# Yifei-Y/Openset-RCNN

Measured on AMD Instinct MI355X. Metric: images/sec at 3x800x1333, R50-FPN, 1/2/4/8 MI355X; mAP_k vs ref, higher is better.
Workload: dtype f16; 1 GPU; VOC-COCO openset_rcnn_R50_FPN_128k.yaml, inference-only, 3x800x1333 uint8 BGR -> padded 800x1344, 1000 proposals/level (4273/img), 1000 dets/img, 50+50 final; batch_per_gpu=16, global_batch=16, parallelism=dp1 (images sharded, no collective), detections_last_step=1600, unknown_detections_last_step=800, known_detections_last_step=800, micro_batch_streams=1, hipgraph=True, ranks=1, distinct_gpus=1, passes_in_flight=4, images_in_flight=64

## Files before the change

### include/osr.h

```cpp
#ifndef OSR_H_
#define OSR_H_

#include <stdint.h>

#ifdef __cplusplus
extern "C" {
#endif

#define OSR_ABI_VERSION 1

typedef int32_t osr_status;
enum {
    OSR_OK = 0,
    OSR_ERR_INVALID_ARG = -1,
    OSR_ERR_UNSUPPORTED = -2,
    OSR_ERR_LAUNCH = -3,
    OSR_ERR_WORKSPACE = -4
};

typedef enum { OSR_F32 = 0, OSR_F16 = 1, OSR_BF16 = 2 } osr_dtype;

#define OSR_MAX_LEVELS 8

int32_t osr_abi_version(void);
// ... 137 lines not shown

int32_t osr_rpn_select_capacity(const osr_rpn_levels* lv, int32_t pre_nms_topk);
int64_t osr_rpn_select_workspace_bytes(const osr_rpn_levels* lv, int32_t n, int32_t pre_nms_topk);
osr_status osr_rpn_select(const osr_rpn_levels* lv, const float* cell_anchors , const float* ctr,
                          const float* deltas, int32_t n, const int32_t* image_hw , int32_t pre_nms_topk,
                          float min_box_size, float* boxes, float* scores, int32_t* src_index, int32_t* batch_idx,
                          int32_t* counts, int32_t* status_flags, void* workspace, int64_t workspace_bytes,
                          void* stream);

osr_status osr_rpn_select_ex(const osr_rpn_levels* lv, const float* cell_anchors, const float* ctr, const float* deltas,
                             int32_t n, const int32_t* image_hw, int32_t pre_nms_topk, float min_box_size,
                             int32_t decode_mode, const float reg_weights[4], float* boxes, float* scores,
                             int32_t* src_index, int32_t* batch_idx, int32_t* level_out, int32_t* counts,
                             int32_t* status_flags, void* workspace, int64_t workspace_bytes, void* stream);

typedef struct osr_pyramid {
    int32_t num_levels;
    int32_t c;
    int32_t h[OSR_MAX_LEVELS];
    int32_t w[OSR_MAX_LEVELS];
    float scale[OSR_MAX_LEVELS];
    const void* data[OSR_MAX_LEVELS];
} osr_pyramid;

osr_status osr_roi_align_fwd(const osr_pyramid* feats, int32_t feat_dtype, int32_t n, const float* boxes,
                             const int32_t* batch_idx, int64_t m, int32_t pooled, int32_t canonical_level,
                             int32_t canonical_size, int32_t min_level, void* out, int32_t out_dtype, void* stream);

osr_status osr_roi_align_fwd_ordered(const osr_pyramid* feats, int32_t feat_dtype, int32_t n, const float* boxes,
                                     const int32_t* batch_idx, int64_t m, int32_t pooled, int32_t canonical_level,
                                     int32_t canonical_size, int32_t min_level, const int32_t* order,
                                     const int32_t* order_nvalid, void* out, int32_t out_dtype, void* stream);
#define OSR_ROI_NO_PADDING_FILL 1
osr_status osr_roi_align_fwd_ordered_ex(const osr_pyramid* feats, int32_t feat_dtype, int32_t n, const float* boxes,
                                        const int32_t* batch_idx, int64_t m, int32_t pooled, int32_t canonical_level,
                                        int32_t canonical_size, int32_t min_level, const int32_t* order,
                                        const int32_t* order_nvalid, int32_t flags, void* out, int32_t out_dtype, void* stream);
#define OSR_ROI_MAX_SAMPLING_RATIO 64
typedef struct osr_roi_options {
    int32_t aligned;
    int32_t sampling_ratio;
} osr_roi_options;
osr_status osr_roi_align_fwd_ordered_opt(const osr_pyramid* feats, int32_t feat_dtype, int32_t n, const float* boxes,
                                         const int32_t* batch_idx, int64_t m, int32_t pooled, int32_t canonical_level,
                                         int32_t canonical_size, int32_t min_level, const int32_t* order,
                                         const int32_t* order_nvalid, int32_t flags, const osr_roi_options* options, void* out,
                                         int32_t out_dtype, void* stream);
int64_t osr_roi_locality_order_workspace_bytes(int32_t n, int64_t m);
osr_status osr_roi_locality_order(const osr_pyramid* feats, int32_t n, const float* boxes, const int32_t* batch_idx, int64_t m,
                                  int32_t canonical_level, int32_t canonical_size, int32_t min_level, int32_t* order,
                                  int32_t* nvalid, void* workspace, int64_t workspace_bytes, void* stream);

osr_status osr_box_predictor_tail(const float* x, int64_t m, int32_t k, const float* w, const float* b,
                                  const float* proposals, const float* ctr, const int32_t* batch_idx,
                                  const int32_t* image_hw, const float reg_weights[4], int32_t mean_type,
                                  float score_thresh, float* pred_deltas, float* pred_iou, float* boxes,
                                  float* score, int32_t* cand, void* stream);

int64_t osr_nms_topk_workspace_bytes(int32_t num_segments, int64_t seg_stride);
osr_status osr_nms_topk(const float* boxes, const float* scores, const int32_t* cls ,
                        const int32_t* cand , int32_t num_segments, int64_t seg_stride,
                        const int32_t* seg_len, float thr, int32_t topk, int32_t* keep, int32_t* keep_count,
                        void* workspace, int64_t workspace_bytes, void* stream);

osr_status osr_gather_rows(const float* src, int64_t seg_stride, int32_t row_elems, const int32_t* keep,
                           const int32_t* keep_count, int32_t num_segments, int32_t topk, float* dst, void* stream);
// ... 272 lines not shown
```

### openset-rcnn_amd/csrc/osr_roi_align.hip

```cpp
#include "osr_common.h"
#include <stdlib.h>

#ifndef RA_MAXC
#define RA_MAXC 32
#endif
#ifndef RA_MAXX
#define RA_MAXX 192
#endif
#ifndef RA_FWD_MAXX
#define RA_FWD_MAXX 96
#endif
#ifndef RA_PAIR
#define RA_PAIR 0
#endif
#ifndef RA_PD1
#define RA_PD1 6
#define RA_PD2 4
#define RA_PD3 2
#define RA_PD4 2
#endif
#ifndef RA_SD1
#define RA_SD1 8
#define RA_SD2 4
#define RA_SD3 3
// ... 2 lines not shown
#endif
#define RA_MAXD 16

struct RaOpt {
    float off;
    int clamp1;
    int sgrid;
};

static bool ra_opt_default(const osr_roi_options* o) { return !o || (o->aligned == 1 && o->sampling_ratio == 0); }
static RaOpt ra_opt_of(const osr_roi_options* o) {
    RaOpt r;
    r.off = (!o || o->aligned) ? 0.5f : 0.f; r.clamp1 = (o && !o->aligned) ? 1 : 0; r.sgrid = o ? o->sampling_ratio : 0;
    return r;
}
#define RA_REQUIRE_OPT(o, name)                                                                                                              \
    OSR_REQUIRE(!(o) || (o)->aligned == 0 || (o)->aligned == 1, OSR_ERR_INVALID_ARG, name ": options: aligned must be 0 or 1, got %d", (o)->aligned); \
    OSR_REQUIRE(!(o) || ((o)->sampling_ratio >= 0 && (o)->sampling_ratio <= OSR_ROI_MAX_SAMPLING_RATIO), OSR_ERR_INVALID_ARG,               \
                name ": options: sampling_ratio must be 0 (adaptive) .. %d, got %d", OSR_ROI_MAX_SAMPLING_RATIO, (o)->sampling_ratio)

struct RoiAlignArgs {
    const void* data[4];
    int h[4], w[4];
    float scale[4];
    int num_levels, c;
    const float* boxes;
    const int* batch_idx;
    long long m;
    int pooled, canonical_level, canonical_size, min_level;
    void* out;
    const int* order;
    const int* order_nvalid;
    int no_pad_fill;
    RaOpt opt;
};

template <class T> struct Vec4;
template <> struct Vec4<float> { typedef float4 type; };
template <> struct Vec4<f16_t> { typedef uint2 type; };
template <> struct Vec4<bf16_t> { typedef uint2 type; };

template <class T> __device__ __forceinline__ void load4(const T* p, float v[4]);
template <> __device__ __forceinline__ void load4<float>(const float* p, float v[4]) {
    float4 t = *reinterpret_cast<const float4*>(p);
    v[0] = t.x; v[1] = t.y; v[2] = t.z; v[3] = t.w;
}
template <> __device__ __forceinline__ void load4<f16_t>(const f16_t* p, float v[4]) {
    typedef f16_t h4 __attribute__((ext_vector_type(4)));
    h4 t = *reinterpret_cast<const h4*>(p);
    v[0] = (float)t[0]; v[1] = (float)t[1]; v[2] = (float)t[2]; v[3] = (float)t[3];
}
template <> __device__ __forceinline__ void load4<bf16_t>(const bf16_t* p, float v[4]) {
    uint2 t = *reinterpret_cast<const uint2*>(p);
    v[0] = __uint_as_float(t.x << 16); v[1] = __uint_as_float(t.x & 0xffff0000u);
    v[2] = __uint_as_float(t.y << 16); v[3] = __uint_as_float(t.y & 0xffff0000u);
}
template <class T> __device__ __forceinline__ void store4(T* p, const float v[4]);
template <> __device__ __forceinline__ void store4<float>(float* p, const float v[4]) {
    *reinterpret_cast<float4*>(p) = make_float4(v[0], v[1], v[2], v[3]);
}
template <> __device__ __forceinline__ void store4<f16_t>(f16_t* p, const float v[4]) {
    typedef f16_t h4 __attribute__((ext_vector_type(4)));
    h4 t = {(f16_t)v[0], (f16_t)v[1], (f16_t)v[2], (f16_t)v[3]};
    *reinterpret_cast<h4*>(p) = t;
}
template <> __device__ __forceinline__ void store4<bf16_t>(bf16_t* p, const float v[4]) {
// ... 169 lines not shown
template <int D, class G, class LoadF, class ConsF>
__device__ __forceinline__ void ra_stream(int n, LoadF load, ConsF cons) {
    G v[D], u[D > 1 ? D - 1 : 1];
    const int q = n / D, r = n - q * D;
    if (q >= 1) {
#pragma unroll
        for (int d = 0; d < D; ++d) load(v[d], d);
        for (int i = 0; i + 1 < q; ++i) {
#pragma unroll
            for (int d = 0; d < D; ++d) { cons(v[d], i * D + d); load(v[d], (i + 1) * D + d); }
        }
    }
#pragma unroll
    for (int d = 0; d < D - 1; ++d) if (d < r) load(u[d], q * D + d);
    if (q >= 1) {
#pragma unroll
        for (int d = 0; d < D; ++d) cons(v[d], (q - 1) * D + d);
    }
#pragma unroll
    for (int d = 0; d < D - 1; ++d) if (d < r) cons(u[d], q * D + d);
}

template <class TO>
__device__ __forceinline__ void ra_store_bins(const ra_f2 (&acc)[7][2], float inv_count, TO* __restrict__ outrow, size_t ostride, bool cok, int P) {
    if (!cok) return;
#pragma unroll
    for (int b = 0; b < 7; ++b)
        if (b < P) {
            const float tot[4] = {acc[b][0][0] * inv_count, acc[b][0][1] * inv_count, acc[b][1][0] * inv_count, acc[b][1][1] * inv_count};
            store4<TO>(outrow + (size_t)b * ostride, tot);
        }
}

template <int NY, class TI, class TO>
__device__ __forceinline__ void ra_bin_row(__amdgpu_buffer_rsrc_t rs, int voff, int base, int istride_b, int sstride_b, int ncol, const RaWaveLds& S,
                                           const float (&wy)[6], float inv_count, TO* __restrict__ outrow, size_t ostride, bool cok, int P) {
    constexpr int D = NY == 1 ? RA_SD1 : NY == 2 ? RA_SD2 : NY == 3 ? RA_SD3 : NY <= 5 ? RA_SD4 : RA_SD6;
    static_assert(D <= RA_MAXD, "S.wfull is padded with RA_MAXD zero rows");
    ra_f2 acc[7][2];
#pragma unroll
    for (int b = 0; b < 7; ++b) { acc[b][0] = ra_f2{0.f, 0.f}; acc[b][1] = ra_f2{0.f, 0.f}; }
    struct Grp { Buf4<TI> p[NY]; };
    ra_stream<D, Grp>(
        ncol,
        [&](Grp& g, int x) {
            const int so = base + x * sstride_b;
#pragma unroll
            for (int j = 0; j < NY; ++j) g.p[j].load(rs, voff, so + j * istride_b);
        },
        [&](Grp& g, int x) {
            ra_f2 c0 = ra_f2{0.f, 0.f}, c1 = ra_f2{0.f, 0.f};
#pragma unroll
            for (int j = 0; j < NY; ++j) {
                ra_f2 lo, hi;
                g.p[j].get(lo, hi);
                const ra_f2 wj = ra_f2{wy[j], wy[j]};
                c0 = __builtin_elementwise_fma(wj, lo, c0);
                c1 = __builtin_elementwise_fma(wj, hi, c1);
            }
            const float4 wa = *reinterpret_cast<const float4*>(&S.wfull[x][0]), wb = *reinterpret_cast<const float4*>(&S.wfull[x][4]);
            const float wv[7] = {wa.x, wa.y, wa.z, wa.w, wb.x, wb.y, wb.z};
#pragma unroll
            for (int b = 0; b < 7; ++b) {
                const ra_f2 wq = ra_f2{wv[b], wv[b]};
                acc[b][0] = __builtin_elementwise_fma(wq, c0, acc[b][0]);
                acc[b][1] = __builtin_elementwise_fma(wq, c1, acc[b][1]);
            }
        });
    ra_store_bins<TO>(acc, inv_count, outrow, ostride, cok, P);
}

template <class T> struct Buf8;
template <int HI, bool FIRST> __device__ __forceinline__ float ra_mix(unsigned packed, float w, float c) {
    float d;
    if (FIRST) {
        if (HI) asm("v_fma_mix_f32 %0, %1, %2, 0 op_sel:[1,0,0] op_sel_hi:[1,0,0]" : "=v"(d) : "v"(packed), "s"(w));
        else asm("v_fma_mix_f32 %0, %1, %2, 0 op_sel_hi:[1,0,0]" : "=v"(d) : "v"(packed), "s"(w));
    } else {
        if (HI) asm("v_fma_mix_f32 %0, %1, %2, %3 op_sel:[1,0,0] op_sel_hi:[1,0,0]" : "=v"(d) : "v"(packed), "s"(w), "v"(c));
        else asm("v_fma_mix_f32 %0, %1, %2, %3 op_sel_hi:[1,0,0]" : "=v"(d) : "v"(packed), "s"(w), "v"(c));
    }
    return d;
}
template <> struct Buf8<f16_t> {
    ra_u32x4 r;
    __device__ __forceinline__ void load(__amdgpu_buffer_rsrc_t rs, int vo, int so) { r = __builtin_amdgcn_raw_buffer_load_b128(rs, vo, so, 0); }
    template <bool FIRST> __device__ __forceinline__ void fma_into(float w, float (&cs)[8]) const {
        _Pragma("unroll") for (int i = 0; i < 4; ++i) {
            cs[2 * i] = ra_mix<0, FIRST>(r[i], w, cs[2 * i]);
            cs[2 * i + 1] = ra_mix<1, FIRST>(r[i], w, cs[2 * i + 1]);
        }
    }
};
template <> struct Buf8<bf16_t> {
    ra_u32x4 r;
    __device__ __forceinline__ void load(__amdgpu_buffer_rsrc_t rs, int vo, int so) { r = __builtin_amdgcn_raw_buffer_load_b128(rs, vo, so, 0); }
    template <bool FIRST> __device__ __forceinline__ void fma_into(float w, float (&cs)[8]) const {
        _Pragma("unroll") for (int i = 0; i < 4; ++i) {
            cs[2 * i] = __builtin_fmaf(__uint_as_float(r[i] << 16), w, FIRST ? 0.f : cs[2 * i]);
            cs[2 * i + 1] = __builtin_fmaf(__uint_as_float(r[i] & 0xffff0000u), w, FIRST ? 0.f : cs[2 * i + 1]);
        }
// ... 24 lines not shown
            for (int j = 0; j < NY; ++j) g.p[j].load(rs, voff, so + j * istride_b);
        },
        [&](Grp& g, int ws) {
            float cs[8];
            g.p[0].template fma_into<true>(wy[0], cs);
#pragma unroll
            for (int j = 1; j < NY; ++j) g.p[j].template fma_into<false>(wy[j], cs);
            const float* wr = &S.wfull[2 * ws + half][0];
            const float4 wa = *reinterpret_cast<const float4*>(wr), wb = *reinterpret_cast<const float4*>(wr + 4);
            const float wv[7] = {wa.x, wa.y, wa.z, wa.w, wb.x, wb.y, wb.z};
#pragma unroll
            for (int b = 0; b < 7; ++b) {
                const ra_f2 wq = ra_f2{wv[b], wv[b]};
#pragma unroll
                for (int q = 0; q < 4; ++q) acc[b][q] = __builtin_elementwise_fma(wq, ra_f2{cs[2 * q], cs[2 * q + 1]}, acc[b][q]);
            }
        });
#pragma unroll
    for (int k2 = 0; k2 < 4; ++k2) {
        float tot[8];
#pragma unroll
        for (int q = 0; q < 4; ++q)
#pragma unroll
            for (int e = 0; e < 2; ++e) {
                const unsigned x = __float_as_uint(acc[2 * k2][q][e]), y = 2 * k2 + 1 < 7 ? __float_as_uint(acc[(2 * k2 + 1) % 7][q][e]) : 0u;
                const auto sw = __builtin_amdgcn_permlane32_swap(x, y, false, false);
                tot[2 * q + e] = (__uint_as_float(sw[0]) + __uint_as_float(sw[1])) * inv_count;
            }
        const int bin = 2 * k2 + half;
        if (cok && bin < P) store8<TO>(outrow + (size_t)bin * ostride, tot);
    }
}

template <class TI, class TO>
__device__ __forceinline__ void ra_bin_row_tall(__amdgpu_buffer_rsrc_t rs, int voff, int base, int istride_b, int sstride_b, int ncol, const RaWaveLds& S,
                                                const float* wrow, int ny, float inv_count, TO* __restrict__ outrow, size_t ostride, bool cok, int P) {
    ra_f2 acc[7][2];
#pragma unroll
    for (int b = 0; b < 7; ++b) { acc[b][0] = ra_f2{0.f, 0.f}; acc[b][1] = ra_f2{0.f, 0.f}; }
    for (int x = 0; x < ncol; ++x) {
        const int so = base + x * sstride_b;
        ra_f2 c0 = ra_f2{0.f, 0.f}, c1 = ra_f2{0.f, 0.f};
        for (int j0 = 0; j0 < ny; j0 += 6) {
            Buf4<TI> v[6];
#pragma unroll
            for (int j = 0; j < 6; ++j) v[j].load(rs, voff, so + min(j0 + j, ny - 1) * istride_b);
#pragma unroll
            for (int j = 0; j < 6; ++j) {
                ra_f2 lo, hi;
                v[j].get(lo, hi);
                const float w1 = j0 + j < ny ? wrow[j0 + j] : 0.f;
                const ra_f2 wj = ra_f2{w1, w1};
                c0 = __builtin_elementwise_fma(wj, lo, c0);
                c1 = __builtin_elementwise_fma(wj, hi, c1);
            }
        }
#pragma unroll
        for (int b = 0; b < 7; ++b) {
            const float w1 = S.wfull[x][b];
            const ra_f2 wq = ra_f2{w1, w1};
            acc[b][0] = __builtin_elementwise_fma(wq, c0, acc[b][0]);
            acc[b][1] = __builtin_elementwise_fma(wq, c1, acc[b][1]);
        }
    }
    ra_store_bins<TO>(acc, inv_count, outrow, ostride, cok, P);
}

#ifndef RA_GATHER_MAXS
#define RA_GATHER_MAXS 3
#endif
#ifndef RA_GATHER_BIN
#define RA_GATHER_BIN 2.0f
#endif
static_assert(RA_GATHER_MAXS >= 2 && RA_GATHER_MAXS <= 3, "gather instantiations exist for S = 1, 2 and 3");
static_assert(4 * RA_GATHER_MAXS <= RA_MAXC, "the taps of a bin are laid over its RA_MAXC table columns");
template <int SG, class TI, class TO>
__device__ __forceinline__ void ra_gather_roi(__amdgpu_buffer_rsrc_t rs, int lane, int sub, int C, int P, int W, const RaWaveLds& S,
                                              float inv_count, TO* __restrict__ out) {
    constexpr int NYG = SG <= 2 ? SG : 1;
    const int pix_b = C * (int)sizeof(TI), row_b = W * pix_b;
    for (int ph = sub; ph < P; ph += RA_WPR) {
        int yo[SG][2]; float wy[SG][2];
#pragma unroll
        for (int i = 0; i < SG; ++i)
#pragma unroll
            for (int t = 0; t < 2; ++t) {
                yo[i][t] = __builtin_amdgcn_readfirstlane(__float_as_int(S.w[0][ph][4 * i + t])) * row_b;
                wy[i][t] = __uint_as_float(__builtin_amdgcn_readfirstlane(__float_as_uint(S.w[0][ph][4 * i + 2 + t])));
            }
        for (int pw = 0; pw < P; ++pw) {
            int xo[SG][2]; float wx[SG][2];
#pragma unroll
            for (int i = 0; i < SG; ++i)
#pragma unroll
                for (int t = 0; t < 2; ++t) {
                    xo[i][t] = __builtin_amdgcn_readfirstlane(__float_as_int(S.w[1][pw][4 * i + t])) * pix_b;
                    wx[i][t] = __uint_as_float(__builtin_amdgcn_readfirstlane(__float_as_uint(S.w[1][pw][4 * i + 2 + t])));
// ... 160 lines not shown
    if (lane < P) {
#pragma unroll
        for (int ax = 0; ax < 2; ++ax) {
            const int lo = S.lo[ax][lane], n = S.n[ax][lane];
            if (n > 0) { lo_l[ax] = lo; hi_l[ax] = lo + n; }
        }
    }
#pragma unroll
    for (int ax = 0; ax < 2; ++ax)
#pragma unroll
        for (int d = 1; d < 8; d <<= 1) {
            lo_l[ax] = min(lo_l[ax], __shfl_xor(lo_l[ax], d, 64));
            hi_l[ax] = max(hi_l[ax], __shfl_xor(hi_l[ax], d, 64));
        }
    int ext_lo[2], ext_n[2];
    bool ax_ok[2];
#pragma unroll
    for (int ax = 0; ax < 2; ++ax) {
        const int l = __builtin_amdgcn_readfirstlane(lo_l[ax]), h = __builtin_amdgcn_readfirstlane(hi_l[ax]);
        ext_lo[ax] = l == 0x7fffffff ? 0 : l;
        ext_n[ax] = l == 0x7fffffff ? 0 : h - l;
        ax_ok[ax] = !fallback && ext_n[ax] <= RA_FWD_MAXX;
    }
    const unsigned long long lvl_bytes = (unsigned long long)H * W * C * sizeof(TI);
#ifndef RA_AXIS_SELECT
#define RA_AXIS_SELECT 1
#endif
    int oa = (!RA_AXIS_SELECT || ext_n[1] <= ext_n[0]) ? 1 : 0;
    if (!ax_ok[oa]) oa ^= 1;

    if (ax_ok[oa] && lvl_bytes < (1ull << 31)) {
        const int ia = oa ^ 1;
        const int os = ext_lo[oa], nstep = ext_n[oa];
        for (int sl = gtid; sl < nstep + RA_MAXD; sl += RA_WPR * 64) {
            const int x = os + sl;
#pragma unroll
            for (int bb = 0; bb < 8; ++bb) {
                float wv = 0.f;
                if (bb < P && sl < nstep) { const int i = x - S.lo[oa][bb]; if (i >= 0 && i < S.n[oa][bb]) wv = S.w[oa][bb][i]; }
                S.wfull[sl][bb] = wv;
            }
        }
        RA_SYNC();
        const float inv_count = 1.0f / count;
        const __amdgpu_buffer_rsrc_t rs = __builtin_amdgcn_make_buffer_rsrc(const_cast<TI*>(feat), 0, (int)lvl_bytes, 0x00020000);
        const int rowstride_b = W * C * (int)sizeof(TI), pix_b = C * (int)sizeof(TI);
        const int istride_b = ia == 0 ? rowstride_b : pix_b, sstride_b = ia == 0 ? pix_b : rowstride_b;
        const size_t ostride = oa == 1 ? (size_t)CE : (size_t)P * CE;
        for (int pb = sub; pb < P; pb += RA_WPR) {
            const int i0 = __builtin_amdgcn_readfirstlane(S.lo[ia][pb]), ni = __builtin_amdgcn_readfirstlane(S.n[ia][pb]);
            float wi[6];
#pragma unroll
            for (int j = 0; j < 6; ++j) wi[j] = __uint_as_float(__builtin_amdgcn_readfirstlane(__float_as_uint(j < ni ? S.w[ia][pb][j] : 0.f)));
            const int base = i0 * istride_b + os * sstride_b;
            if (RA_PAIR && sizeof(TI) == 2 && C % 8 == 0 && ni >= 1 && ni <= 4 && nstep > 0) {
                const int half = lane >> 5;
                for (int cb0 = 0; cb0 < C; cb0 += 256) {
                    const int c0 = cb0 + (lane & 31) * 8;
                    const bool cok = c0 < C;
                    const int voff = (cok ? c0 : 0) * (int)sizeof(TI) + half * sstride_b;
                    TO* outrow = out + (size_t)pb * (oa == 1 ? (size_t)P * CE : (size_t)CE) + RA_CBASE(c0);
                    switch (ni) {
                        case 1: ra_bin_row_pair<1, TI, TO>(rs, voff, base, istride_b, sstride_b, nstep, S, half, wi, inv_count, outrow, ostride, cok, P); break;
                        case 2: ra_bin_row_pair<2, TI, TO>(rs, voff, base, istride_b, sstride_b, nstep, S, half, wi, inv_count, outrow, ostride, cok, P); break;
                        case 3: ra_bin_row_pair<3, TI, TO>(rs, voff, base, istride_b, sstride_b, nstep, S, half, wi, inv_count, outrow, ostride, cok, P); break;
                        default: ra_bin_row_pair<4, TI, TO>(rs, voff, base, istride_b, sstride_b, nstep, S, half, wi, inv_count, outrow, ostride, cok, P); break;
                    }
                }
                continue;
            }
            for (int cb0 = 0; cb0 < C; cb0 += 256) {
                const int c0 = cb0 + lane * 4;
                const bool cok = c0 < C;
                const int voff = (cok ? c0 : 0) * (int)sizeof(TI);
                TO* outrow = out + (size_t)pb * (oa == 1 ? (size_t)P * CE : (size_t)CE) + RA_CBASE(c0);
                switch (nstep > 0 ? (ni > 6 ? 7 : ni) : 0) {
                    case 1: ra_bin_row<1, TI, TO>(rs, voff, base, istride_b, sstride_b, nstep, S, wi, inv_count, outrow, ostride, cok, P); break;
                    case 2: ra_bin_row<2, TI, TO>(rs, voff, base, istride_b, sstride_b, nstep, S, wi, inv_count, outrow, ostride, cok, P); break;
                    case 3: ra_bin_row<3, TI, TO>(rs, voff, base, istride_b, sstride_b, nstep, S, wi, inv_count, outrow, ostride, cok, P); break;
                    case 4: ra_bin_row<4, TI, TO>(rs, voff, base, istride_b, sstride_b, nstep, S, wi, inv_count, outrow, ostride, cok, P); break;
                    case 5: ra_bin_row<5, TI, TO>(rs, voff, base, istride_b, sstride_b, nstep, S, wi, inv_count, outrow, ostride, cok, P); break;
                    case 6: ra_bin_row<6, TI, TO>(rs, voff, base, istride_b, sstride_b, nstep, S, wi, inv_count, outrow, ostride, cok, P); break;
                    case 7: ra_bin_row_tall<TI, TO>(rs, voff, base, istride_b, sstride_b, nstep, S, S.w[ia][pb], ni, inv_count, outrow, ostride, cok, P); break;
                    default: {
                        const float z[4] = {0.f, 0.f, 0.f, 0.f};
                        if (cok) for (int q = 0; q < P; ++q) store4<TO>(outrow + (size_t)q * ostride, z);
                    }
                }
            }
        }
        return;
    }

    for (int ph = sub; ph < P; ph += RA_WPR) {
        for (int c0 = lane * 4; c0 < C; c0 += 256) {
            for (int pw = 0; pw < P; ++pw) {
                float acc[4] = {0.f, 0.f, 0.f, 0.f};
                if (!fallback) {
                    const int y0 = S.lo[0][ph], ny = S.n[0][ph], x0 = S.lo[1][pw], nx = S.n[1][pw];
                    for (int j = 0; j < ny; ++j) {
                        const float wy = S.w[0][ph][j];
                        const TI* row = feat + ((size_t)(y0 + j) * W + x0) * C + c0;
                        for (int i = 0; i < nx; ++i) {
                            float v[4];
                            load4<TI>(row + (size_t)i * C, v);
                            const float wgt = wy * S.w[1][pw][i];
                            acc[0] += wgt * v[0]; acc[1] += wgt * v[1]; acc[2] += wgt * v[2]; acc[3] += wgt * v[3];
                        }
                    }
                } else {
                    for (int iy = 0; iy < gh; ++iy) {
                        int yl, yh; float hy, ly;
                        if (!axis_sample(sh, ph, bh, iy, gh, H, &yl, &yh, &hy, &ly)) continue;
                        for (int ix = 0; ix < gw; ++ix) {
                            int xl, xh; float hx, lx;
                            if (!axis_sample(sw, pw, bw, ix, gw, W, &xl, &xh, &hx, &lx)) continue;
// ... 22 lines not shown
    switch (out_dtype) {
        case OSR_F32: hipLaunchKernelGGL((roi_align_kernel<TI, float, OPT>), grid, block, 0, st, a); break;
        case OSR_F16: hipLaunchKernelGGL((roi_align_kernel<TI, f16_t, OPT>), grid, block, 0, st, a); break;
        default: hipLaunchKernelGGL((roi_align_kernel<TI, bf16_t, OPT>), grid, block, 0, st, a); break;
    }
    OSR_CHECK_LAUNCH("osr_roi_align_fwd");
    return OSR_OK;
}

static osr_status roi_align_fwd_impl(const osr_pyramid* f, int32_t feat_dtype, int32_t n, const float* boxes,
                                     const int32_t* batch_idx, int64_t m, int32_t pooled, int32_t canonical_level,
                                     int32_t canonical_size, int32_t min_level, const int32_t* order,
                                     const int32_t* order_nvalid, void* out, int32_t out_dtype, void* stream, int32_t flags = 0,
                                     const osr_roi_options* opt = nullptr) {
    OSR_REQUIRE(f && boxes && batch_idx && out, OSR_ERR_INVALID_ARG, "osr_roi_align_fwd: null pointer");
    RA_REQUIRE_OPT(opt, "osr_roi_align_fwd");
    OSR_REQUIRE(f->num_levels >= 1 && f->num_levels <= 4, OSR_ERR_INVALID_ARG, "osr_roi_align_fwd: 1..4 levels, got %d", f->num_levels);
    OSR_REQUIRE(pooled >= 1 && pooled <= 7, OSR_ERR_UNSUPPORTED, "osr_roi_align_fwd: pooled size 1..7, got %d", pooled);
    OSR_REQUIRE(f->c > 0 && f->c % 4 == 0, OSR_ERR_UNSUPPORTED, "osr_roi_align_fwd: channels must be a multiple of 4, got %d", f->c);
    OSR_REQUIRE(osr_dtype_ok(feat_dtype) && osr_dtype_ok(out_dtype), OSR_ERR_INVALID_ARG, "osr_roi_align_fwd: bad dtype");
    OSR_REQUIRE(n >= 1 && m >= 0 && m < (1ll << 31), OSR_ERR_INVALID_ARG, "osr_roi_align_fwd: bad n/m");
    OSR_REQUIRE(canonical_size > 0, OSR_ERR_INVALID_ARG, "osr_roi_align_fwd: canonical_size must be > 0");
    if (m == 0) return OSR_OK;
    RoiAlignArgs a;
    for (int l = 0; l < 4; ++l) {
        int s = l < f->num_levels ? l : 0;
        OSR_REQUIRE(f->data[s] && f->h[s] > 0 && f->w[s] > 0, OSR_ERR_INVALID_ARG, "osr_roi_align_fwd: bad level %d", s);
        a.data[l] = f->data[s]; a.h[l] = f->h[s]; a.w[l] = f->w[s]; a.scale[l] = f->scale[s];
    }
    a.num_levels = f->num_levels; a.c = f->c; a.boxes = boxes; a.batch_idx = batch_idx; a.m = m;
    a.pooled = pooled; a.canonical_level = canonical_level; a.canonical_size = canonical_size; a.min_level = min_level;
    a.out = out; a.order = order; a.order_nvalid = order ? order_nvalid : nullptr;
    a.no_pad_fill = (flags & OSR_ROI_NO_PADDING_FILL) ? 1 : 0;
    a.opt = ra_opt_of(opt);
    hipStream_t st = (hipStream_t)stream;
    if (ra_opt_default(opt)) {
        switch (feat_dtype) {
            case OSR_F32: return launch_out<float, false>(a, out_dtype, st);
            case OSR_F16: return launch_out<f16_t, false>(a, out_dtype, st);
            default: return launch_out<bf16_t, false>(a, out_dtype, st);
        }
    }
    switch (feat_dtype) {
        case OSR_F32: return launch_out<float, true>(a, out_dtype, st);
        case OSR_F16: return launch_out<f16_t, true>(a, out_dtype, st);
        default: return launch_out<bf16_t, true>(a, out_dtype, st);
    }
}

extern "C" osr_status osr_roi_align_fwd_ordered(const osr_pyramid* f, int32_t feat_dtype, int32_t n, const float* boxes,
                                                const int32_t* batch_idx, int64_t m, int32_t pooled, int32_t canonical_level,
                                                int32_t canonical_size, int32_t min_level, const int32_t* order,
                                                const int32_t* order_nvalid, void* out, int32_t out_dtype, void* stream) {
    return roi_align_fwd_impl(f, feat_dtype, n, boxes, batch_idx, m, pooled, canonical_level, canonical_size, min_level, order, order_nvalid,
                              out, out_dtype, stream);
}

extern "C" osr_status osr_roi_align_fwd_ordered_ex(const osr_pyramid* f, int32_t feat_dtype, int32_t n, const float* boxes,
                                                   const int32_t* batch_idx, int64_t m, int32_t pooled, int32_t canonical_level,
                                                   int32_t canonical_size, int32_t min_level, const int32_t* order,
                                                   const int32_t* order_nvalid, int32_t flags, void* out, int32_t out_dtype, void* stream) {
    OSR_REQUIRE((flags & ~OSR_ROI_NO_PADDING_FILL) == 0, OSR_ERR_INVALID_ARG, "osr_roi_align_fwd_ordered_ex: unknown flag bits 0x%x", flags);
    return roi_align_fwd_impl(f, feat_dtype, n, boxes, batch_idx, m, pooled, canonical_level, canonical_size, min_level, order, order_nvalid,
                              out, out_dtype, stream, flags);
}

extern "C" osr_status osr_roi_align_fwd_ordered_opt(const osr_pyramid* f, int32_t feat_dtype, int32_t n, const float* boxes,
                                                    const int32_t* batch_idx, int64_t m, int32_t pooled, int32_t canonical_level,
                                                    int32_t canonical_size, int32_t min_level, const int32_t* order,
                                                    const int32_t* order_nvalid, int32_t flags, const osr_roi_options* options, void* out,
                                                    int32_t out_dtype, void* stream) {
    OSR_REQUIRE((flags & ~OSR_ROI_NO_PADDING_FILL) == 0, OSR_ERR_INVALID_ARG, "osr_roi_align_fwd_ordered_opt: unknown flag bits 0x%x", flags);
    return roi_align_fwd_impl(f, feat_dtype, n, boxes, batch_idx, m, pooled, canonical_level, canonical_size, min_level, order, order_nvalid,
                              out, out_dtype, stream, flags, options);
}

extern "C" osr_status osr_roi_align_fwd(const osr_pyramid* f, int32_t feat_dtype, int32_t n, const float* boxes,
                                        const int32_t* batch_idx, int64_t m, int32_t pooled, int32_t canonical_level,
                                        int32_t canonical_size, int32_t min_level, void* out, int32_t out_dtype,
                                        void* stream) {
    return osr_roi_align_fwd_ordered(f, feat_dtype, n, boxes, batch_idx, m, pooled, canonical_level, canonical_size, min_level, nullptr, nullptr,
                                     out, out_dtype, stream);
}

#define RA_BUCKETS 128

struct RoiOrderArgs {
    int h[4], w[4];
    float scale[4];
    int num_levels, n;
    const float* boxes;
    const int* batch_idx;
    long long m;
    int canonical_level, canonical_size, min_level;
    int* bucket;
    int* counts;
    int* order;
};

__device__ __forceinline__ int ra_bucket_of(const RoiOrderArgs& a, long long r) {
    const int b = a.batch_idx[r];
    if (b < 0 || b >= a.n) return a.n * RA_BUCKETS;
    const float4 bx = *reinterpret_cast<const float4*>(a.boxes + r * 4);
    float sz = sqrtf((bx.z - bx.x) * (bx.w - bx.y));
    float lvf = floorf((float)a.canonical_level + log2f(sz / (float)a.canonical_size + 1e-8f));
// ... 601 lines not shown
```

### openset-rcnn_amd/host/ops.py

```python
from __future__ import annotations

import ctypes as C
from typing import List, Optional, Sequence, Tuple

import torch

from . import _lib
from ._lib import ConvParams, OsrError, Pyramid, RpnLevels, check

_DT = {torch.float32: _lib.OSR_F32, torch.float16: _lib.OSR_F16, torch.bfloat16: _lib.OSR_BF16}


def _p(t: Optional[torch.Tensor]):
    return None if t is None else C.c_void_p(t.data_ptr())


def _stream():
    return C.c_void_p(torch.cuda.current_stream().cuda_stream)


def _need(t: torch.Tensor, dtype=None, name="tensor"):
    if not t.is_cuda:
        raise OsrError(f"{name} must live on the GPU (got {t.device}); the HIP path has no CPU fallback")
    if dtype is not None and t.dtype != dtype:
# ... 782 lines not shown
                       canonical_level: int = 4, canonical_size: int = 224, min_level: int = 2) -> torch.Tensor:
    lib = _lib.load()
    _need(boxes, torch.float32, "boxes"); _need(batch_idx, torch.int32, "batch_idx")
    py = _pyramid(feats, scales)
    m, n = boxes.shape[0], feats[0].shape[0]
    order = torch.empty((m + 1,), dtype=torch.int32, device=boxes.device)
    nb = int(lib.osr_roi_locality_order_workspace_bytes(n, m))
    ws = torch.empty((max(nb, 4),), dtype=torch.uint8, device=boxes.device)
    check(lib.osr_roi_locality_order(C.byref(py), n, _p(boxes), _p(batch_idx), m, canonical_level, canonical_size, min_level, _p(order),
                                     C.c_void_p(order.data_ptr() + 4 * m), _p(ws), nb, _stream()), "osr_roi_locality_order")
    return order


MAX_SAMPLING_RATIO = 64


def check_pooler_options(aligned, sampling_ratio) -> Tuple[bool, int]:
    if not isinstance(aligned, (bool, int)) or aligned not in (0, 1):
        raise ValueError(f"RoIAlign: aligned must be True (POOLER_TYPE 'ROIAlignV2') or False ('ROIAlign'), got {aligned!r}")
    if isinstance(sampling_ratio, bool) or not isinstance(sampling_ratio, int) or not 0 <= sampling_ratio <= MAX_SAMPLING_RATIO:
        raise ValueError(f"RoIAlign: sampling_ratio must be an integer 0 .. {MAX_SAMPLING_RATIO} (0 = adaptive grid, S > 0 = S x S samples per bin), "
                         f"got {sampling_ratio!r}")
    return bool(aligned), int(sampling_ratio)


def _roi_options(aligned, sampling_ratio):
    aligned, sampling_ratio = check_pooler_options(aligned, sampling_ratio)
    return C.byref(_lib.RoiOptions(int(aligned), sampling_ratio))


def roi_align(feats: List[torch.Tensor], scales: Sequence[float], boxes: torch.Tensor, batch_idx: torch.Tensor,
              pooled: int = 7, out_dtype: Optional[torch.dtype] = None, canonical_level: int = 4, canonical_size: int = 224,
              min_level: int = 2, order: Optional[torch.Tensor] = None, fill_padding: bool = True, aligned: bool = True,
              sampling_ratio: int = 0) -> torch.Tensor:
    lib = _lib.load()
    opt = _roi_options(aligned, sampling_ratio)
    _need(boxes, torch.float32, "boxes"); _need(batch_idx, torch.int32, "batch_idx")
    py = _pyramid(feats, scales)
    m = boxes.shape[0]
    if order is None and ROI_LOCALITY_ORDER and m > 0:
        order = roi_locality_order(feats, scales, boxes, batch_idx, canonical_level, canonical_size, min_level)
    nvalid = None
    if order is not None:
        _need(order, torch.int32, "order")
        assert order.numel() in (m, m + 1)
        if order.numel() == m + 1:
            nvalid = C.c_void_p(order.data_ptr() + 4 * m)
    out_dtype = out_dtype or feats[0].dtype
    out = torch.empty((m, pooled, pooled, py.c), dtype=out_dtype, device=boxes.device)
    check(lib.osr_roi_align_fwd_ordered_opt(C.byref(py), _DT[feats[0].dtype], feats[0].shape[0], _p(boxes), _p(batch_idx), m, pooled,
                                            canonical_level, canonical_size, min_level, _p(order), nvalid, 0 if fill_padding else 1, opt,
                                            _p(out), _DT[out_dtype], _stream()), "osr_roi_align_fwd")
    return out


def box_predictor_tail(x, w, b, proposals, ctr, batch_idx, image_hw, reg_weights=(10.0, 10.0, 5.0, 5.0), mean_type=0,
                       score_thresh=0.05):
    lib = _lib.load()
    for t, nme in ((x, "x"), (w, "w"), (b, "b"), (proposals, "proposals"), (ctr, "ctr")):
        _need(t, torch.float32, nme)
    _need(batch_idx, torch.int32, "batch_idx"); _need(image_hw, torch.int32, "image_hw")
    m, k = x.shape
    dev = x.device
    pd = torch.empty((m, 4), dtype=torch.float32, device=dev)
    pi = torch.empty((m,), dtype=torch.float32, device=dev)
    bx = torch.empty((m, 4), dtype=torch.float32, device=dev)
    sc = torch.empty((m,), dtype=torch.float32, device=dev)
    cd = torch.empty((m,), dtype=torch.int32, device=dev)
    rw = (C.c_float * 4)(*[float(v) for v in reg_weights])
    check(lib.osr_box_predictor_tail(_p(x), m, k, _p(w), _p(b), _p(proposals), _p(ctr), _p(batch_idx), _p(image_hw), rw, mean_type,
                                     float(score_thresh), _p(pd), _p(pi), _p(bx), _p(sc), _p(cd), _stream()), "osr_box_predictor_tail")
    return dict(pred_deltas=pd, pred_iou=pi, boxes=bx, score=sc, cand=cd)


def nms_topk(boxes, scores, cls, cand, num_segments: int, seg_stride: int, seg_len, thr: float, topk: int):
    lib = _lib.load()
    _need(boxes, torch.float32, "boxes"); _need(scores, torch.float32, "scores"); _need(seg_len, torch.int32, "seg_len")
    if cls is not None:
        _need(cls, torch.int32, "cls")
    if cand is not None:
        _need(cand, torch.int32, "cand")
    dev = boxes.device
    wsb = lib.osr_nms_topk_workspace_bytes(num_segments, seg_stride)
    if wsb < 0:
# ... 825 lines not shown
```

Baseline: 1594 images/sec.

## Use two-bin sliding window accumulation in RoIAlign column pass for f16

In the separable RoIAlign column pass, each column's interpolation weights are usually nonzero for at most two adjacent output bins. A per-column starting-bin index is stored in the LDS weight table, and when every column satisfies the two-adjacent-bins property, a specialized path is used. That path accumulates into only a current and next bin and parks finished bins in a vector, instead of doing seven FMAs per column. This cuts ALU work and LDS reads, at the cost of an extra validation pass and barrier, more template instantiations, and possible register pressure from the 32-wide parked-bin vector.

```diff
diff --git a/include/osr.h b/include/osr.h
--- a/include/osr.h
+++ b/include/osr.h
@@ -193,6 +193,7 @@
                                      int32_t canonical_size, int32_t min_level, const int32_t* order,
                                      const int32_t* order_nvalid, void* out, int32_t out_dtype, void* stream);
 #define OSR_ROI_NO_PADDING_FILL 1
+#define OSR_ROI_DENSE_BINS 2
 osr_status osr_roi_align_fwd_ordered_ex(const osr_pyramid* feats, int32_t feat_dtype, int32_t n, const float* boxes,
                                         const int32_t* batch_idx, int64_t m, int32_t pooled, int32_t canonical_level,
                                         int32_t canonical_size, int32_t min_level, const int32_t* order,
diff --git a/openset-rcnn_amd/csrc/osr_roi_align.hip b/openset-rcnn_amd/csrc/osr_roi_align.hip
--- a/openset-rcnn_amd/csrc/osr_roi_align.hip
+++ b/openset-rcnn_amd/csrc/osr_roi_align.hip
@@ -58,6 +58,7 @@
     const int* order;
     const int* order_nvalid;
     int no_pad_fill;
+    int dense_bins;
     RaOpt opt;
 };
 
@@ -293,7 +294,51 @@
         }
 }
 
-template <int NY, class TI, class TO>
+typedef float ra_f32 __attribute__((ext_vector_type(32)));
+struct RaWindow {
+    ra_f32 bins;
+    ra_f2 cur[2], nxt[2];
+    float4 tn;
+    int cb;
+    __device__ __forceinline__ RaWindow(const RaWaveLds& S) : cb(0) {
+        cur[0] = cur[1] = nxt[0] = nxt[1] = ra_f2{0.f, 0.f};
+#pragma unroll
+        for (int i = 0; i < 32; ++i) bins[i] = 0.f;
+        tn = *reinterpret_cast<const float4*>(&S.wfull[0][4]);
+    }
+    __device__ __forceinline__ void park(int b, const ra_f2 (&v)[2]) {
+        bins[4 * b] = v[0][0]; bins[4 * b + 1] = v[0][1]; bins[4 * b + 2] = v[1][0]; bins[4 * b + 3] = v[1][1];
+    }
+    __device__ __forceinline__ void step(const RaWaveLds& S, int x, ra_f2 c0, ra_f2 c1) {
+        const float4 t = tn;
+        tn = *reinterpret_cast<const float4*>(&S.wfull[x + 1][4]);
+        const int b0 = __builtin_amdgcn_readfirstlane(__float_as_int(t.w));
+        const int w0i = __builtin_amdgcn_readfirstlane(__float_as_int(t.x)), w1i = __builtin_amdgcn_readfirstlane(__float_as_int(t.y));
+        const float w0 = __int_as_float(w0i), w1 = __int_as_float(w1i);
+        while (cb < b0) {
+            park(cb, cur);
+            cur[0] = nxt[0]; cur[1] = nxt[1]; nxt[0] = nxt[1] = ra_f2{0.f, 0.f};
+            ++cb;
+        }
+        if (w0i != 0) {
+            asm volatile("");
+            const ra_f2 wq = ra_f2{w0, w0};
+            cur[0] = __builtin_elementwise_fma(wq, c0, cur[0]); cur[1] = __builtin_elementwise_fma(wq, c1, cur[1]);
+        }
+        if (w1i != 0) {
+            asm volatile("");
+            const ra_f2 wq = ra_f2{w1, w1};
+            nxt[0] = __builtin_elementwise_fma(wq, c0, nxt[0]); nxt[1] = __builtin_elementwise_fma(wq, c1, nxt[1]);
+        }
+    }
+    __device__ __forceinline__ void finish(ra_f2 (&acc)[7][2]) {
+        park(cb, cur); park(cb + 1, nxt);
+#pragma unroll
+        for (int b = 0; b < 7; ++b) { acc[b][0] = ra_f2{bins[4 * b], bins[4 * b + 1]}; acc[b][1] = ra_f2{bins[4 * b + 2], bins[4 * b + 3]}; }
+    }
+};
+
+template <int NY, bool WIN, class TI, class TO>
 __device__ __forceinline__ void ra_bin_row(__amdgpu_buffer_rsrc_t rs, int voff, int base, int istride_b, int sstride_b, int ncol, const RaWaveLds& S,
                                            const float (&wy)[6], float inv_count, TO* __restrict__ outrow, size_t ostride, bool cok, int P) {
     constexpr int D = NY == 1 ? RA_SD1 : NY == 2 ? RA_SD2 : NY == 3 ? RA_SD3 : NY <= 5 ? RA_SD4 : RA_SD6;
@@ -301,6 +346,7 @@
     ra_f2 acc[7][2];
 #pragma unroll
     for (int b = 0; b < 7; ++b) { acc[b][0] = ra_f2{0.f, 0.f}; acc[b][1] = ra_f2{0.f, 0.f}; }
+    RaWindow win(S);
     struct Grp { Buf4<TI> p[NY]; };
     ra_stream<D, Grp>(
         ncol,
@@ -319,6 +365,10 @@
                 c0 = __builtin_elementwise_fma(wj, lo, c0);
                 c1 = __builtin_elementwise_fma(wj, hi, c1);
             }
+            if (WIN) {
+                win.step(S, x, c0, c1);
+                return;
+            }
             const float4 wa = *reinterpret_cast<const float4*>(&S.wfull[x][0]), wb = *reinterpret_cast<const float4*>(&S.wfull[x][4]);
             const float wv[7] = {wa.x, wa.y, wa.z, wa.w, wb.x, wb.y, wb.z};
 #pragma unroll
@@ -328,6 +378,7 @@
                 acc[b][1] = __builtin_elementwise_fma(wq, c1, acc[b][1]);
             }
         });
+    if (WIN) win.finish(acc);
     ra_store_bins<TO>(acc, inv_count, outrow, ostride, cok, P);
 }
 
@@ -418,12 +469,13 @@
     }
 }
 
-template <class TI, class TO>
+template <bool WIN, class TI, class TO>
 __device__ __forceinline__ void ra_bin_row_tall(__amdgpu_buffer_rsrc_t rs, int voff, int base, int istride_b, int sstride_b, int ncol, const RaWaveLds& S,
                                                 const float* wrow, int ny, float inv_count, TO* __restrict__ outrow, size_t ostride, bool cok, int P) {
     ra_f2 acc[7][2];
 #pragma unroll
     for (int b = 0; b < 7; ++b) { acc[b][0] = ra_f2{0.f, 0.f}; acc[b][1] = ra_f2{0.f, 0.f}; }
+    RaWindow win(S);
     for (int x = 0; x < ncol; ++x) {
         const int so = base + x * sstride_b;
         ra_f2 c0 = ra_f2{0.f, 0.f}, c1 = ra_f2{0.f, 0.f};
@@ -441,6 +493,10 @@
                 c1 = __builtin_elementwise_fma(wj, hi, c1);
             }
         }
+        if (WIN) {
+            win.step(S, x, c0, c1);
+            continue;
+        }
 #pragma unroll
         for (int b = 0; b < 7; ++b) {
             const float w1 = S.wfull[x][b];
@@ -449,6 +505,7 @@
             acc[b][1] = __builtin_elementwise_fma(wq, c1, acc[b][1]);
         }
     }
+    if (WIN) win.finish(acc);
     ra_store_bins<TO>(acc, inv_count, outrow, ostride, cok, P);
 }
 
@@ -675,16 +732,39 @@
     if (ax_ok[oa] && lvl_bytes < (1ull << 31)) {
         const int ia = oa ^ 1;
         const int os = ext_lo[oa], nstep = ext_n[oa];
+        constexpr bool kWin = sizeof(TI) == 2 && !RA_PAIR;
+        bool wbad = a.dense_bins != 0 || !kWin;
         for (int sl = gtid; sl < nstep + RA_MAXD; sl += RA_WPR * 64) {
             const int x = os + sl;
+            int b0 = -1, bu = 6;
 #pragma unroll
             for (int bb = 0; bb < 8; ++bb) {
                 float wv = 0.f;
-                if (bb < P && sl < nstep) { const int i = x - S.lo[oa][bb]; if (i >= 0 && i < S.n[oa][bb]) wv = S.w[oa][bb][i]; }
+                if (bb < P && sl < nstep) {
+                    const int i = x - S.lo[oa][bb], nb = S.n[oa][bb];
+                    if (i >= 0 && i < nb) wv = S.w[oa][bb][i];
+                    if (nb > 0 && i < nb) bu = min(bu, bb);
+                }
                 S.wfull[sl][bb] = wv;
-            }
+                if (wv != 0.f) {
+                    if (b0 < 0) b0 = bb;
+                    if (bb > b0 + 1) wbad = true;
+                }
+            }
+            S.wfull[sl][7] = __int_as_float(b0 < 0 ? bu : b0);
         }
         RA_SYNC();
+        for (int sl = gtid; sl < nstep; sl += RA_WPR * 64)
+            if (sl > 0 && __float_as_int(S.wfull[sl][7]) < __float_as_int(S.wfull[sl - 1][7])) wbad = true;
+        const bool win = kWin && !RA_ANY(wbad);
+        if (win) {
+            for (int sl = gtid; sl < nstep + RA_MAXD; sl += RA_WPR * 64) {
+                const int b0 = __float_as_int(S.wfull[sl][7]);
+                const float w0 = S.wfull[sl][b0], w1 = b0 < 6 ? S.wfull[sl][b0 + 1] : 0.f;
+                S.wfull[sl][4] = w0; S.wfull[sl][5] = w1;
+            }
+            RA_SYNC();
+        }
         const float inv_count = 1.0f / count;
         const __amdgpu_buffer_rsrc_t rs = __builtin_amdgcn_make_buffer_rsrc(const_cast<TI*>(feat), 0, (int)lvl_bytes, 0x00020000);
         const int rowstride_b = W * C * (int)sizeof(TI), pix_b = C * (int)sizeof(TI);
@@ -718,13 +798,27 @@
                 const int voff = (cok ? c0 : 0) * (int)sizeof(TI);
                 TO* outrow = out + (size_t)pb * (oa == 1 ? (size_t)P * CE : (size_t)CE) + RA_CBASE(c0);
                 switch (nstep > 0 ? (ni > 6 ? 7 : ni) : 0) {
-                    case 1: ra_bin_row<1, TI, TO>(rs, voff, base, istride_b, sstride_b, nstep, S, wi, inv_count, outrow, ostride, cok, P); break;
-                    case 2: ra_bin_row<2, TI, TO>(rs, voff, base, istride_b, sstride_b, nstep, S, wi, inv_count, outrow, ostride, cok, P); break;
-                    case 3: ra_bin_row<3, TI, TO>(rs, voff, base, istride_b, sstride_b, nstep, S, wi, inv_count, outrow, ostride, cok, P); break;
-                    case 4: ra_bin_row<4, TI, TO>(rs, voff, base, istride_b, sstride_b, nstep, S, wi, inv_count, outrow, ostride, cok, P); break;
-                    case 5: ra_bin_row<5, TI, TO>(rs, voff, base, istride_b, sstride_b, nstep, S, wi, inv_count, outrow, ostride, cok, P); break;
-                    case 6: ra_bin_row<6, TI, TO>(rs, voff, base, istride_b, sstride_b, nstep, S, wi, inv_count, outrow, ostride, cok, P); break;
-                    case 7: ra_bin_row_tall<TI, TO>(rs, voff, base, istride_b, sstride_b, nstep, S, S.w[ia][pb], ni, inv_count, outrow, ostride, cok, P); break;
+                    case 1: if (kWin && win) ra_bin_row<1, true, TI, TO>(rs, voff, base, istride_b, sstride_b, nstep, S, wi, inv_count, outrow, ostride, cok, P);
+                            else ra_bin_row<1, false, TI, TO>(rs, voff, base, istride_b, sstride_b, nstep, S, wi, inv_count, outrow, ostride, cok, P);
+                            break;
+                    case 2: if (kWin && win) ra_bin_row<2, true, TI, TO>(rs, voff, base, istride_b, sstride_b, nstep, S, wi, inv_count, outrow, ostride, cok, P);
+                            else ra_bin_row<2, false, TI, TO>(rs, voff, base, istride_b, sstride_b, nstep, S, wi, inv_count, outrow, ostride, cok, P);
+                            break;
+                    case 3: if (kWin && win) ra_bin_row<3, true, TI, TO>(rs, voff, base, istride_b, sstride_b, nstep, S, wi, inv_count, outrow, ostride, cok, P);
+                            else ra_bin_row<3, false, TI, TO>(rs, voff, base, istride_b, sstride_b, nstep, S, wi, inv_count, outrow, ostride, cok, P);
+                            break;
+                    case 4: if (kWin && win) ra_bin_row<4, true, TI, TO>(rs, voff, base, istride_b, sstride_b, nstep, S, wi, inv_count, outrow, ostride, cok, P);
+                            else ra_bin_row<4, false, TI, TO>(rs, voff, base, istride_b, sstride_b, nstep, S, wi, inv_count, outrow, ostride, cok, P);
+                            break;
+                    case 5: if (kWin && win) ra_bin_row<5, true, TI, TO>(rs, voff, base, istride_b, sstride_b, nstep, S, wi, inv_count, outrow, ostride, cok, P);
+                            else ra_bin_row<5, false, TI, TO>(rs, voff, base, istride_b, sstride_b, nstep, S, wi, inv_count, outrow, ostride, cok, P);
+                            break;
+                    case 6: if (kWin && win) ra_bin_row<6, true, TI, TO>(rs, voff, base, istride_b, sstride_b, nstep, S, wi, inv_count, outrow, ostride, cok, P);
+                            else ra_bin_row<6, false, TI, TO>(rs, voff, base, istride_b, sstride_b, nstep, S, wi, inv_count, outrow, ostride, cok, P);
+                            break;
+                    case 7: if (kWin && win) ra_bin_row_tall<true, TI, TO>(rs, voff, base, istride_b, sstride_b, nstep, S, S.w[ia][pb], ni, inv_count, outrow, ostride, cok, P);
+                            else ra_bin_row_tall<false, TI, TO>(rs, voff, base, istride_b, sstride_b, nstep, S, S.w[ia][pb], ni, inv_count, outrow, ostride, cok, P);
+                            break;
                     default: {
                         const float z[4] = {0.f, 0.f, 0.f, 0.f};
                         if (cok) for (int q = 0; q < P; ++q) store4<TO>(outrow + (size_t)q * ostride, z);
@@ -813,6 +907,7 @@
     a.pooled = pooled; a.canonical_level = canonical_level; a.canonical_size = canonical_size; a.min_level = min_level;
     a.out = out; a.order = order; a.order_nvalid = order ? order_nvalid : nullptr;
     a.no_pad_fill = (flags & OSR_ROI_NO_PADDING_FILL) ? 1 : 0;
+    a.dense_bins = (flags & OSR_ROI_DENSE_BINS) ? 1 : 0;
     a.opt = ra_opt_of(opt);
     hipStream_t st = (hipStream_t)stream;
     if (ra_opt_default(opt)) {
@@ -841,7 +936,7 @@
                                                    const int32_t* batch_idx, int64_t m, int32_t pooled, int32_t canonical_level,
                                                    int32_t canonical_size, int32_t min_level, const int32_t* order,
                                                    const int32_t* order_nvalid, int32_t flags, void* out, int32_t out_dtype, void* stream) {
-    OSR_REQUIRE((flags & ~OSR_ROI_NO_PADDING_FILL) == 0, OSR_ERR_INVALID_ARG, "osr_roi_align_fwd_ordered_ex: unknown flag bits 0x%x", flags);
+    OSR_REQUIRE((flags & ~(OSR_ROI_NO_PADDING_FILL | OSR_ROI_DENSE_BINS)) == 0, OSR_ERR_INVALID_ARG, "osr_roi_align_fwd_ordered_ex: unknown flag bits 0x%x", flags);
     return roi_align_fwd_impl(f, feat_dtype, n, boxes, batch_idx, m, pooled, canonical_level, canonical_size, min_level, order, order_nvalid,
                               out, out_dtype, stream, flags);
 }
@@ -851,7 +946,7 @@
                                                     int32_t canonical_size, int32_t min_level, const int32_t* order,
                                                     const int32_t* order_nvalid, int32_t flags, const osr_roi_options* options, void* out,
                                                     int32_t out_dtype, void* stream) {
-    OSR_REQUIRE((flags & ~OSR_ROI_NO_PADDING_FILL) == 0, OSR_ERR_INVALID_ARG, "osr_roi_align_fwd_ordered_opt: unknown flag bits 0x%x", flags);
+    OSR_REQUIRE((flags & ~(OSR_ROI_NO_PADDING_FILL | OSR_ROI_DENSE_BINS)) == 0, OSR_ERR_INVALID_ARG, "osr_roi_align_fwd_ordered_opt: unknown flag bits 0x%x", flags);
     return roi_align_fwd_impl(f, feat_dtype, n, boxes, batch_idx, m, pooled, canonical_level, canonical_size, min_level, order, order_nvalid,
                               out, out_dtype, stream, flags, options);
 }
diff --git a/openset-rcnn_amd/host/ops.py b/openset-rcnn_amd/host/ops.py
--- a/openset-rcnn_amd/host/ops.py
+++ b/openset-rcnn_amd/host/ops.py
@@ -838,7 +838,7 @@
 def roi_align(feats: List[torch.Tensor], scales: Sequence[float], boxes: torch.Tensor, batch_idx: torch.Tensor,
               pooled: int = 7, out_dtype: Optional[torch.dtype] = None, canonical_level: int = 4, canonical_size: int = 224,
               min_level: int = 2, order: Optional[torch.Tensor] = None, fill_padding: bool = True, aligned: bool = True,
-              sampling_ratio: int = 0) -> torch.Tensor:
+              sampling_ratio: int = 0, dense_bins: bool = False) -> torch.Tensor:
     lib = _lib.load()
     opt = _roi_options(aligned, sampling_ratio)
     _need(boxes, torch.float32, "boxes"); _need(batch_idx, torch.int32, "batch_idx")
@@ -855,7 +855,8 @@
     out_dtype = out_dtype or feats[0].dtype
     out = torch.empty((m, pooled, pooled, py.c), dtype=out_dtype, device=boxes.device)
     check(lib.osr_roi_align_fwd_ordered_opt(C.byref(py), _DT[feats[0].dtype], feats[0].shape[0], _p(boxes), _p(batch_idx), m, pooled,
-                                            canonical_level, canonical_size, min_level, _p(order), nvalid, 0 if fill_padding else 1, opt,
+                                            canonical_level, canonical_size, min_level, _p(order), nvalid,
+                                            (0 if fill_padding else 1) | (2 if dense_bins else 0), opt,
                                             _p(out), _DT[out_dtype], _stream()), "osr_roi_align_fwd")
     return out
 
```

Measured after the change: 1592 images/sec. No clear change (-0.1%).
